# Bitcoin-Wildlife-Sanctuary/recursive-stwo

Hardware: AMD Instinct MI355X
Metric: recursive proofs verified/sec (higher is better)
Workload: dtype u32 (M31 modular integers)

## Files before the change

### recursive-stwo_amd/csrc/poseidon2.hpp

```cpp
#pragma once
#include "field.hpp"

namespace rsv {

struct State16 {
    uint32_t s[16];
};

#define RSV_RC_FULL_INIT { \
    {0x768bab52, 0x70e0ab7d, 0x3d266c8a, 0x6da42045, 0x600fef22, 0x41dace6b, 0x64f9bdd4, 0x5d42d4fe, \
     0x76b1516d, 0x6fc9a717, 0x70ac4fb6, 0x00194ef6, 0x22b644e2, 0x1f7916d5, 0x47581be2, 0x2710a123}, \
    {0x6284e867, 0x018d3afe, 0x5df99ef3, 0x4c1e467b, 0x566f6abc, 0x2994e427, 0x538a6d42, 0x5d7bf2cf, \
     0x7fda2dab, 0x0fd854c4, 0x46922fca, 0x3d7763a1, 0x19fd05ca, 0x0a4bbb43, 0x15075851, 0x3d903d76}, \
    {0x2d290ff7, 0x40809fa0, 0x59dac6ec, 0x127927a2, 0x6bbf0ea0, 0x0294140f, 0x24742976, 0x6e84c081, \
     0x22484f4a, 0x354cae59, 0x0453ffe1, 0x3f47a3cc, 0x0088204e, 0x6066e109, 0x3b7c4b80, 0x6b55665d}, \
    {0x3bc4b897, 0x735bf378, 0x508daf42, 0x1884fc2b, 0x7214f24c, 0x7498be0a, 0x1a60e640, 0x3303f928, \
     0x29b46376, 0x5c96bb68, 0x65d097a5, 0x1d358e9f, 0x4a9a9017, 0x4724cf76, 0x347af70f, 0x1e77e59a}, \
    {0x57090613, 0x1fa42108, 0x17bbef50, 0x1ff7e11c, 0x047b24ca, 0x4e140275, 0x4fa086f5, 0x079b309c, \
     0x1159bd47, 0x6d37e4e5, 0x075d8dce, 0x12121ca0, 0x7f6a7c40, 0x68e182ba, 0x5493201b, 0x0444a80e}, \
    {0x0064f4c6, 0x6467abe6, 0x66975762, 0x2af68f9b, 0x345b33be, 0x1b70d47f, 0x053db717, 0x381189cb, \
     0x43b915f8, 0x20df3694, 0x0f459d26, 0x77a0e97b, 0x2f73e739, 0x1876c2f9, 0x65a0e29a, 0x4cabefbe}, \
    {0x5abd1268, 0x4d34a760, 0x12771799, 0x69a0c9ac, 0x39091e55, 0x7f611cd0, 0x3af055da, 0x7ac0bbdf, \
     0x6e0f3a24, 0x41e3b6f7, 0x49b3756d, 0x568bc538, 0x20c079d8, 0x1701c72c, 0x7670dc6c, 0x5a439035}, \
    {0x7c93e00e, 0x561fbb4d, 0x1178907b, 0x02737406, 0x32fb24f1, 0x6323b60a, 0x6ab12418, 0x42c99cea, \
     0x155a0b97, 0x53d1c6aa, 0x2bd20347, 0x279b3d73, 0x4f5f3c70, 0x0245af6c, 0x238359d3, 0x49966a59}}
__constant__ __attribute__((aligned(64))) uint32_t RC_FULL[8][16] = RSV_RC_FULL_INIT;
constexpr uint32_t RC_FULL_K[8][16] = RSV_RC_FULL_INIT;

#define RSV_RC_PARTIAL_INIT { \
   0x7f7ec4bf, 0x0421926f, 0x5198e669, 0x34db3148, 0x4368bafd, \
                                        0x66685c7f, 0x78d3249a, 0x60187881, 0x76dad67a, 0x0690b437, \
                                        0x1ea95311, 0x40e5369a, 0x38f103fc, 0x1d226a21, 0, 0}
__constant__ __attribute__((aligned(64))) uint32_t RC_PARTIAL[16] = RSV_RC_PARTIAL_INIT;
constexpr uint32_t RC_PARTIAL_K[16] = RSV_RC_PARTIAL_INIT;

__device__ __forceinline__ uint32_t pow5_ref(uint32_t x) {
    uint32_t x2 = m_sqr(x);
    return m_mul(m_sqr(x2), x);
}

__device__ __forceinline__ void mds4_ref(uint32_t& x0, uint32_t& x1, uint32_t& x2, uint32_t& x3) {
    uint32_t t0 = m_add(x0, x1), t1 = m_add(x2, x3);
    uint32_t t2 = m_add(m_dbl(x1), t1), t3 = m_add(m_dbl(x3), t0);
    uint32_t t4 = m_add(m_shl(t1, 2), t3), t5 = m_add(m_shl(t0, 2), t2);
    x0 = m_add(t3, t5);
    x1 = t5;
    x2 = m_add(t2, t4);
    x3 = t4;
}

__device__ __forceinline__ void mds16_ref(uint32_t* s) {
#pragma unroll
    for (int g = 0; g < 4; g++) mds4_ref(s[4 * g], s[4 * g + 1], s[4 * g + 2], s[4 * g + 3]);
#pragma unroll
    for (int j = 0; j < 4; j++) {
        uint32_t sum = m_add(m_add(s[j], s[j + 4]), m_add(s[j + 8], s[j + 12]));
#pragma unroll
        for (int g = 0; g < 4; g++) s[4 * g + j] = m_add(s[4 * g + j], sum);
    }
}

template <bool PACE>
struct PermT {
    static __device__ __forceinline__ uint64_t add64(uint64_t a, uint64_t b) {
        uint64_t d;
        asm("v_lshl_add_u64 %0, %1, 0, %2" : "=v"(d) : "v"(a), "v"(b));
        return d;
    }
    template <int SH>
    static __device__ __forceinline__ uint64_t shl_add64(uint64_t a, uint64_t b) {
        uint64_t d;
        asm("v_lshl_add_u64 %0, %1, %3, %2" : "=v"(d) : "v"(a), "v"(b), "n"(SH));
        return d;
    }
    static __device__ __forceinline__ uint32_t opaque(uint32_t k) {
        uint32_t r;
        asm volatile("s_mov_b32 %0, %1" : "=s"(r) : "n"(k));
        return r;
    }
    static __device__ __forceinline__ uint64_t opaque64(uint64_t k) {
        return (uint64_t)opaque((uint32_t)(k >> 32)) << 32 | opaque((uint32_t)k);
    }
    static __device__ __forceinline__ uint64_t mul64(uint32_t a, uint32_t b_uniform) {
        uint64_t d, carry;
        if constexpr (PACE) asm("v_mad_u64_u32 %0, %1, %2, %3, 0\n\ts_nop 0" : "=v"(d), "=s"(carry) : "v"(a), "s"(b_uniform));
        else asm("v_mad_u64_u32 %0, %1, %2, %3, 0" : "=v"(d), "=s"(carry) : "v"(a), "s"(b_uniform));
        return d;
    }
    static __device__ __forceinline__ uint64_t mad64(uint32_t a, uint32_t b_uniform, uint64_t c) {
        uint64_t d, carry;
        if constexpr (PACE) asm("v_mad_u64_u32 %0, %1, %2, %3, %4\n\ts_nop 0" : "=v"(d), "=s"(carry) : "v"(a), "s"(b_uniform), "v"(c));
        else asm("v_mad_u64_u32 %0, %1, %2, %3, %4" : "=v"(d), "=s"(carry) : "v"(a), "s"(b_uniform), "v"(c));
        return d;
    }
    static __device__ __forceinline__ uint64_t mad64s(int32_t a, int32_t b, uint64_t c_uniform) {
        uint64_t d, carry;
        if constexpr (PACE) asm("v_mad_i64_i32 %0, %1, %2, %3, %4\n\ts_nop 0" : "=v"(d), "=s"(carry) : "v"(a), "v"(b), "s"(c_uniform));
        else asm("v_mad_i64_i32 %0, %1, %2, %3, %4" : "=v"(d), "=s"(carry) : "v"(a), "v"(b), "s"(c_uniform));
        return d;
    }
    static __device__ __forceinline__ uint64_t sqr64s(int32_t a, uint64_t c_uniform) {
        uint64_t d, carry;
        if constexpr (PACE) asm("v_mad_i64_i32 %0, %1, %2, %2, %3\n\ts_nop 0" : "=v"(d), "=s"(carry) : "v"(a), "s"(c_uniform));
        else asm("v_mad_i64_i32 %0, %1, %2, %2, %3" : "=v"(d), "=s"(carry) : "v"(a), "s"(c_uniform));
        return d;
    }
    static __device__ __forceinline__ uint32_t dbl32(uint32_t x) {
        uint32_t d;
        asm("v_add_u32 %0, %1, %1" : "=v"(d) : "v"(x));
        return d;
    }
    static __device__ __forceinline__ uint32_t fold2(uint64_t V) {
        uint32_t r = (uint32_t)(V >> 32) + ((uint32_t)V >> 1);
        return r;
    }

    static constexpr uint64_t KP = 0 - ((uint64_t)P << 32);
    static constexpr uint64_t KN = 0 - ((uint64_t)P << 31), KQ = (uint64_t)P << 31;
    struct SboxK {
        uint64_t kp, kn, kq;
    };
    static __device__ __forceinline__ SboxK sbox_k() { return {opaque64(KP), opaque64(KN), opaque64(KQ)}; }
    static constexpr uint32_t CENTRE = 1u << 30;
    static constexpr uint32_t centred(uint32_t rc) { return (uint32_t)(((uint64_t)rc + CENTRE) % P); }

    static __device__ __forceinline__ uint32_t pow5c(int32_t x, const SboxK& k) {
        const int32_t xx = (int32_t)dbl32((uint32_t)x);
        const int32_t s1 = (int32_t)fold2(mad64s(xx, x, k.kp));
        const uint64_t V2 = sqr64s(s1, k.kn);
        uint32_t c4 = __builtin_amdgcn_alignbit((uint32_t)(V2 >> 32), (uint32_t)V2, 31) + ((uint32_t)V2 & P);
        if constexpr (PACE) asm volatile("s_nop 0" : "+v"(c4));
        return fold2(mad64s(xx, (int32_t)c4, k.kq));
    }

    static __device__ __forceinline__ void mds4_2x(uint32_t k2, uint32_t k4, uint32_t x0, uint32_t x1, uint32_t x2, uint32_t x3,
                                            uint64_t& y0, uint64_t& y1, uint64_t& y2, uint64_t& y3) {
        uint64_t T0 = mad64(x0, k2, mul64(x1, k2));
        uint64_t T1 = mad64(x2, k2, mul64(x3, k2));
        uint64_t T2 = mad64(x1, k4, T1);
        uint64_t T3 = mad64(x3, k4, T0);
        uint64_t T4 = shl_add64<2>(T1, T3);
        uint64_t T5 = shl_add64<2>(T0, T2);
        y0 = add64(T3, T5);
        y1 = T5;
        y2 = add64(T2, T4);
        y3 = T4;
    }

    static __device__ __forceinline__ void mds16_2x(uint32_t k2, uint32_t k4, const uint32_t* s, uint64_t* V) {
    #pragma unroll
        for (int g = 0; g < 4; g++)
            mds4_2x(k2, k4, s[4 * g], s[4 * g + 1], s[4 * g + 2], s[4 * g + 3], V[4 * g], V[4 * g + 1], V[4 * g + 2], V[4 * g + 3]);
    #pragma unroll
        for (int j = 0; j < 4; j++) {
            uint64_t sum = add64(add64(V[j], V[j + 4]), add64(V[j + 8], V[j + 12]));
    #pragma unroll
            for (int g = 0; g < 4; g++) V[4 * g + j] = add64(V[4 * g + j], sum);
        }
    }

    static constexpr uint32_t HI_FULL = 160, HI_PARTIAL = 1u << 18;
    template <uint32_t RC, uint32_t HI>
    static __device__ __forceinline__ int32_t centre_rc(uint32_t t) {
        static_assert(HI < P - RC, "round constant too close to P for the fused reduction");
        constexpr uint32_t c = P - RC;
        static_assert((uint64_t)P + HI - c <= 0x7FFFFFFFull, "t - c leaves the int32 range");
        const int32_t a = (int32_t)(t - c);
        const uint32_t q = (uint32_t)(a >> 31) ^ 0xC0000000u;
        return (int32_t)((uint32_t)a + q);
    }

    template <int R, int I>
    static __device__ __forceinline__ void sbox_full(const uint64_t* V, uint32_t* s, const SboxK& k) {
        s[I] = pow5c(centre_rc<centred(RC_FULL_K[R][I]), HI_FULL>(fold2(V[I])), k);
        if constexpr (I + 1 < 16) sbox_full<R, I + 1>(V, s, k);
    }
    template <int I>
    static __device__ __forceinline__ void sbox_full4(uint32_t* s, const SboxK& k) {
        s[I] = pow5c(centre_rc<centred(RC_FULL_K[4][I]), HI_PARTIAL>(s[I]), k);
        if constexpr (I + 1 < 16) sbox_full4<I + 1>(s, k);
    }

    template <int R>
    static __device__ __forceinline__ void partial_round(uint32_t* s, uint32_t k2, uint32_t k6, const uint32_t* kd, const SboxK& k) {
        uint32_t u0 = pow5c(centre_rc<centred(RC_PARTIAL_K[R]), HI_PARTIAL>(s[0]), k);
        uint64_t a = mul64(u0, k2), b = mul64(s[1], k2);
    #pragma unroll
        for (int i = 2; i < 16; i += 2) { a = mad64(s[i], k2, a); b = mad64(s[i + 1], k2, b); }
        uint64_t sum2 = add64(a, b);
        s[0] = fold2(mad64(u0, k6, sum2));
    #pragma unroll
        for (int i = 1; i < 16; i++) s[i] = fold2(mad64(s[i], kd[i], sum2));
    }

    template <int R>
    static __device__ __forceinline__ void partial_pair(uint32_t* s, uint32_t k2, uint32_t k6, uint32_t k30, const uint32_t* kd,
                                                        const uint32_t* kq, const SboxK& k) {
        uint32_t u0 = pow5c(centre_rc<centred(RC_PARTIAL_K[R]), HI_PARTIAL>(s[0]), k);
        uint64_t a = mul64(u0, k2), b = mul64(s[1], k2);
    #pragma unroll
        for (int i = 2; i < 16; i += 2) { a = mad64(s[i], k2, a); b = mad64(s[i + 1], k2, b); }
        uint64_t sum2 = add64(a, b);
        const uint32_t s0 = fold2(mad64(u0, k6, sum2));
        const uint32_t sf = fold2(sum2);
        u0 = pow5c(centre_rc<centred(RC_PARTIAL_K[R + 1]), HI_PARTIAL>(s0), k);
        a = mul64(u0, k2); b = mul64(s[1], kd[1]);
    #pragma unroll
        for (int i = 2; i < 16; i += 2) { a = mad64(s[i], kd[i], a); b = mad64(s[i + 1], kd[i + 1], b); }
        a = mad64(sf, k30, a);
        sum2 = add64(a, b);
        s[0] = fold2(mad64(u0, k6, sum2));
    #pragma unroll
        for (int i = 1; i < 16; i++) s[i] = fold2(mad64(s[i], kq[i], mad64(sf, kd[i], sum2)));
    }

    static __device__ __forceinline__ void poseidon2_rounds(uint32_t* s, uint32_t k2, uint32_t k4) {
        uint64_t V[16];
        const uint32_t k6 = opaque(6);
        const SboxK k5 = sbox_k();
        mds16_2x(k2, k4, s, V);
        sbox_full<0, 0>(V, s, k5); mds16_2x(k2, k4, s, V);
        sbox_full<1, 0>(V, s, k5); mds16_2x(k2, k4, s, V);
        sbox_full<2, 0>(V, s, k5); mds16_2x(k2, k4, s, V);
        sbox_full<3, 0>(V, s, k5); mds16_2x(k2, k4, s, V);
    #pragma unroll
        for (int i = 0; i < 16; i++) s[i] = fold2(V[i]);
        uint32_t kd[16];
        kd[0] = k6;
    #define RSV_KD(i) kd[i] = opaque(4u << (i));
        RSV_KD(1) RSV_KD(2) RSV_KD(3) RSV_KD(4) RSV_KD(5) RSV_KD(6) RSV_KD(7) RSV_KD(8)
        RSV_KD(9) RSV_KD(10) RSV_KD(11) RSV_KD(12) RSV_KD(13) RSV_KD(14) RSV_KD(15)
    #undef RSV_KD
        uint32_t kq[16];
        kq[0] = 0;
    #pragma unroll
        for (int i = 1; i < 8; i++) kq[i] = kd[2 * i + 1];
    #define RSV_KQ(i) kq[i] = opaque(8u << (2 * (i)));
        RSV_KQ(8) RSV_KQ(9) RSV_KQ(10) RSV_KQ(11) RSV_KQ(12) RSV_KQ(13) RSV_KQ(14)
    #undef RSV_KQ
        kq[15] = k4;
        const uint32_t k30 = opaque(30);
        partial_round<0>(s, k2, k6, kd, k5);
        partial_pair<1>(s, k2, k6, k30, kd, kq, k5);  partial_pair<3>(s, k2, k6, k30, kd, kq, k5);  partial_pair<5>(s, k2, k6, k30, kd, kq, k5);
        partial_pair<7>(s, k2, k6, k30, kd, kq, k5);  partial_pair<9>(s, k2, k6, k30, kd, kq, k5);  partial_pair<11>(s, k2, k6, k30, kd, kq, k5);
        partial_round<13>(s, k2, k6, kd, k5);
        sbox_full4<0>(s, k5);      mds16_2x(k2, k4, s, V);
        sbox_full<5, 0>(V, s, k5); mds16_2x(k2, k4, s, V);
        sbox_full<6, 0>(V, s, k5); mds16_2x(k2, k4, s, V);
        sbox_full<7, 0>(V, s, k5);
    }

    static __device__ __forceinline__ void poseidon2_inline(uint32_t* s) {
        const uint32_t k2 = opaque(2), k4 = opaque(4);
        poseidon2_rounds(s, k2, k4);
        uint64_t V[16];
        mds16_2x(k2, k4, s, V);
    #pragma unroll
        for (int i = 0; i < 16; i++) {
            uint32_t t = fold2(V[i]);
            s[i] = min(t, t - P);
        }
    }

    template <bool HI>
    static __device__ __forceinline__ void poseidon2_inline_half(uint32_t* s, uint32_t* out8) {
        const uint32_t k2 = opaque(2), k4 = opaque(4);
        poseidon2_rounds(s, k2, k4);
        uint64_t V[16];
    #pragma unroll
        for (int g = 0; g < 4; g++)
            mds4_2x(k2, k4, s[4 * g], s[4 * g + 1], s[4 * g + 2], s[4 * g + 3], V[4 * g], V[4 * g + 1], V[4 * g + 2], V[4 * g + 3]);
        if constexpr (HI) {
    #pragma unroll
            for (int j = 0; j < 4; j++) {
                const uint64_t sum = add64(add64(V[j], V[j + 4]), add64(V[j + 8], V[j + 12]));
                const uint32_t t0 = fold2(add64(V[8 + j], sum)), t1 = fold2(add64(V[12 + j], sum));
                out8[j] = min(t0, t0 - P);
                out8[4 + j] = min(t1, t1 - P);
            }
        } else {
    #pragma unroll
            for (int j = 0; j < 4; j++) {
                const uint64_t sum = add64(add64(V[j], V[j + 4]), add64(V[j + 8], V[j + 12]));
                const uint32_t t0 = fold2(add64(V[j], sum)), t1 = fold2(add64(V[4 + j], sum));
                out8[j] = min(t0, t0 - P);
                out8[4 + j] = min(t1, t1 - P);
            }
        }
    }
};
__device__ __forceinline__ void poseidon2_inline(uint32_t* s) { PermT<true>::poseidon2_inline(s); }

#ifdef RSV_COUNT_PERMS
__device__ unsigned long long g_perm_counter[16];
__shared__ unsigned s_perm_tag;
#define RSV_TAG(k) do { if (threadIdx.x == 0) s_perm_tag = (k); __syncthreads(); } while (0)
__device__ __forceinline__ void count_perm_call() {
    const unsigned long long m = __ballot(1);
    if ((threadIdx.x & 63u) == (unsigned)__builtin_ctzll(m)) {
        atomicAdd(&g_perm_counter[2 * (s_perm_tag & 7u)], (unsigned long long)__builtin_popcountll(m));
        atomicAdd(&g_perm_counter[2 * (s_perm_tag & 7u) + 1], 1ull);
    }
}
#else
#define RSV_TAG(k) do { } while (0)
__device__ __forceinline__ void count_perm_call() {}
#endif

__device__ __noinline__ State16 poseidon2(State16 st) {
    count_perm_call();
    poseidon2_inline(st.s);
    return st;
}

struct Hash8 {
    uint32_t w[8];
};
__device__ __forceinline__ State16 join(const Hash8& l, const Hash8& r) {
    State16 st;
#pragma unroll
    for (int i = 0; i < 8; i++) { st.s[i] = l.w[i]; st.s[8 + i] = r.w[i]; }
    return st;
}
__device__ __forceinline__ Hash8 rate_of(const State16& st) {
    Hash8 h;
#pragma unroll
    for (int i = 0; i < 8; i++) h.w[i] = st.s[i];
    return h;
}
__device__ __forceinline__ Hash8 cap_of(const State16& st) {
    Hash8 h;
#pragma unroll
    for (int i = 0; i < 8; i++) h.w[i] = st.s[8 + i];
    return h;
}
__device__ __forceinline__ Hash8 zero8() {
    Hash8 h;
#pragma unroll
    for (int i = 0; i < 8; i++) h.w[i] = 0;
    return h;
}
template <bool HI, bool PACE>
__device__ __noinline__ Hash8 poseidon2_half_t(State16 st) {
    count_perm_call();
    Hash8 h;
    PermT<PACE>::template poseidon2_inline_half<HI>(st.s, h.w);
    return h;
}
struct RowRC {
    uint32_t f[8];
};
__device__ __forceinline__ RowRC load_row_rc(uint32_t i) {
    RowRC k;
#pragma unroll
    for (int r = 0; r < 8; r++) k.f[r] = RC_FULL[r][i];
    return k;
}
template <bool HI>
__device__ __noinline__ Hash8 poseidon2_row_half(State16 st);
__device__ __noinline__ State16 poseidon2_row_state(State16 st);
__shared__ uint32_t s_row_rc[8][16];
template <int PACE>
__device__ __forceinline__ void row_rc_init() {
    if constexpr (PACE == 2) {
        if (threadIdx.x < 128) s_row_rc[threadIdx.x >> 4][threadIdx.x & 15u] = RC_FULL[threadIdx.x >> 4][threadIdx.x & 15u];
        __syncthreads();
    }
}
constexpr int FORM_ROW = 2;
template <int PACE = 1>
__device__ __forceinline__ Hash8 poseidon2_half(State16 st, uint32_t hi) {
    if constexpr (PACE == FORM_ROW) return hi ? poseidon2_row_half<true>(st) : poseidon2_row_half<false>(st);
    else return hi ? poseidon2_half_t<true, PACE != 0>(st) : poseidon2_half_t<false, PACE != 0>(st);
}
template <int PACE = 1>
__device__ __forceinline__ State16 poseidon2_full(State16 st) {
    if constexpr (PACE == FORM_ROW) return poseidon2_row_state(st);
    else return poseidon2(st);
}
template <int PACE>
__device__ __forceinline__ uint32_t vlane() { return PACE == FORM_ROW ? threadIdx.x >> 4 : threadIdx.x; }
template <int PACE = 1>
__device__ __forceinline__ Hash8 perm_rate(const Hash8& l, const Hash8& r) { return poseidon2_half<PACE>(join(l, r), 0u); }
template <int PACE = 1>
__device__ __forceinline__ Hash8 perm_cap(const Hash8& l, const Hash8& r) { return poseidon2_half<PACE>(join(l, r), 1u); }
__device__ __forceinline__ bool hash_eq(const Hash8& a, const Hash8& b) {
    uint32_t d = 0;
#pragma unroll
    for (int i = 0; i < 8; i++) d |= a.w[i] ^ b.w[i];
    return d == 0;
}

}
```

Baseline: 2.207 million.

## Restructure Poseidon2 external MDS as column-sum plus per-group M4

Rewrites the 16-wide external MDS so the doubled column sums across the four groups are computed first. Each group then applies a multiply-free M4 (adds and shifts) to x*2 plus the column sum. The s-box of each group now runs right after that group's MDS, so only four 64-bit accumulators are live at a time instead of sixteen. The goal is fewer multiplies and lower register pressure in the full rounds. The cost is a different instruction mix and reliance on M4 being linear to keep the result identical.

Result: faster. 2.238 million (median of 6 runs) (+1.4%).

```diff
diff --git a/recursive-stwo_amd/csrc/poseidon2.hpp b/recursive-stwo_amd/csrc/poseidon2.hpp
--- a/recursive-stwo_amd/csrc/poseidon2.hpp
+++ b/recursive-stwo_amd/csrc/poseidon2.hpp
@@ -133,32 +133,28 @@
         return fold2(mad64s(xx, (int32_t)c4, k.kq));
     }
 
-    static __device__ __forceinline__ void mds4_2x(uint32_t k2, uint32_t k4, uint32_t x0, uint32_t x1, uint32_t x2, uint32_t x3,
-                                            uint64_t& y0, uint64_t& y1, uint64_t& y2, uint64_t& y3) {
-        uint64_t T0 = mad64(x0, k2, mul64(x1, k2));
-        uint64_t T1 = mad64(x2, k2, mul64(x3, k2));
-        uint64_t T2 = mad64(x1, k4, T1);
-        uint64_t T3 = mad64(x3, k4, T0);
-        uint64_t T4 = shl_add64<2>(T1, T3);
-        uint64_t T5 = shl_add64<2>(T0, T2);
-        y0 = add64(T3, T5);
-        y1 = T5;
-        y2 = add64(T2, T4);
-        y3 = T4;
-    }
-
-    static __device__ __forceinline__ void mds16_2x(uint32_t k2, uint32_t k4, const uint32_t* s, uint64_t* V) {
-    #pragma unroll
-        for (int g = 0; g < 4; g++)
-            mds4_2x(k2, k4, s[4 * g], s[4 * g + 1], s[4 * g + 2], s[4 * g + 3], V[4 * g], V[4 * g + 1], V[4 * g + 2], V[4 * g + 3]);
-    #pragma unroll
-        for (int j = 0; j < 4; j++) {
-            uint64_t sum = add64(add64(V[j], V[j + 4]), add64(V[j + 8], V[j + 12]));
-    #pragma unroll
-            for (int g = 0; g < 4; g++) V[4 * g + j] = add64(V[4 * g + j], sum);
+    static __device__ __forceinline__ void colsums_2x(uint32_t k2, const uint32_t* s, uint64_t* X2) {
+    #pragma unroll
+        for (int j = 0; j < 4; j++) X2[j] = mul64(s[j], k2);
+    #pragma unroll
+        for (int g = 1; g < 4; g++) {
+    #pragma unroll
+            for (int j = 0; j < 4; j++) X2[j] = mad64(s[4 * g + j], k2, X2[j]);
         }
     }
-
+    static __device__ __forceinline__ void mds4(uint64_t z0, uint64_t z1, uint64_t z2, uint64_t z3,
+                                                uint64_t& y0, uint64_t& y1, uint64_t& y2, uint64_t& y3) {
+        uint64_t t0 = add64(z0, z1), t1 = add64(z2, z3);
+        uint64_t t2 = shl_add64<1>(z1, t1), t3 = shl_add64<1>(z3, t0);
+        uint64_t t4 = shl_add64<2>(t1, t3), t5 = shl_add64<2>(t0, t2);
+        y0 = add64(t3, t5);
+        y1 = t5;
+        y2 = add64(t2, t4);
+        y3 = t4;
+    }
+    static __device__ __forceinline__ void mds_group_2x(uint32_t k2, const uint64_t* X2, const uint32_t* x, uint64_t* V) {
+        mds4(mad64(x[0], k2, X2[0]), mad64(x[1], k2, X2[1]), mad64(x[2], k2, X2[2]), mad64(x[3], k2, X2[3]), V[0], V[1], V[2], V[3]);
+    }
     static constexpr uint32_t HI_FULL = 160, HI_PARTIAL = 1u << 18;
     template <uint32_t RC, uint32_t HI>
     static __device__ __forceinline__ int32_t centre_rc(uint32_t t) {
@@ -170,10 +166,30 @@
         return (int32_t)((uint32_t)a + q);
     }
 
-    template <int R, int I>
+    template <int R, int I, int END = 16>
     static __device__ __forceinline__ void sbox_full(const uint64_t* V, uint32_t* s, const SboxK& k) {
         s[I] = pow5c(centre_rc<centred(RC_FULL_K[R][I]), HI_FULL>(fold2(V[I])), k);
-        if constexpr (I + 1 < 16) sbox_full<R, I + 1>(V, s, k);
+        if constexpr (I + 1 < END) sbox_full<R, I + 1, END>(V, s, k);
+    }
+    template <int R>
+    static __device__ __forceinline__ void mds_sbox(uint32_t k2, uint32_t* s, const SboxK& k) {
+        uint64_t X2[4], V[16];
+        colsums_2x(k2, s, X2);
+        mds_group_2x(k2, X2, s, V);           sbox_full<R, 0, 4>(V, s, k);
+        mds_group_2x(k2, X2, s + 4, V + 4);   sbox_full<R, 4, 8>(V, s, k);
+        mds_group_2x(k2, X2, s + 8, V + 8);   sbox_full<R, 8, 12>(V, s, k);
+        mds_group_2x(k2, X2, s + 12, V + 12); sbox_full<R, 12, 16>(V, s, k);
+    }
+    static __device__ __forceinline__ void mds_fold(uint32_t k2, uint32_t* s) {
+        uint64_t X2[4];
+        colsums_2x(k2, s, X2);
+    #pragma unroll
+        for (int g = 0; g < 4; g++) {
+            uint64_t V[4];
+            mds_group_2x(k2, X2, s + 4 * g, V);
+    #pragma unroll
+            for (int j = 0; j < 4; j++) s[4 * g + j] = fold2(V[j]);
+        }
     }
     template <int I>
     static __device__ __forceinline__ void sbox_full4(uint32_t* s, const SboxK& k) {
@@ -215,16 +231,13 @@
     }
 
     static __device__ __forceinline__ void poseidon2_rounds(uint32_t* s, uint32_t k2, uint32_t k4) {
-        uint64_t V[16];
         const uint32_t k6 = opaque(6);
         const SboxK k5 = sbox_k();
-        mds16_2x(k2, k4, s, V);
-        sbox_full<0, 0>(V, s, k5); mds16_2x(k2, k4, s, V);
-        sbox_full<1, 0>(V, s, k5); mds16_2x(k2, k4, s, V);
-        sbox_full<2, 0>(V, s, k5); mds16_2x(k2, k4, s, V);
-        sbox_full<3, 0>(V, s, k5); mds16_2x(k2, k4, s, V);
-    #pragma unroll
-        for (int i = 0; i < 16; i++) s[i] = fold2(V[i]);
+        mds_sbox<0>(k2, s, k5);
+        mds_sbox<1>(k2, s, k5);
+        mds_sbox<2>(k2, s, k5);
+        mds_sbox<3>(k2, s, k5);
+        mds_fold(k2, s);
         uint32_t kd[16];
         kd[0] = k6;
     #define RSV_KD(i) kd[i] = opaque(4u << (i));
@@ -244,47 +257,34 @@
         partial_pair<1>(s, k2, k6, k30, kd, kq, k5);  partial_pair<3>(s, k2, k6, k30, kd, kq, k5);  partial_pair<5>(s, k2, k6, k30, kd, kq, k5);
         partial_pair<7>(s, k2, k6, k30, kd, kq, k5);  partial_pair<9>(s, k2, k6, k30, kd, kq, k5);  partial_pair<11>(s, k2, k6, k30, kd, kq, k5);
         partial_round<13>(s, k2, k6, kd, k5);
-        sbox_full4<0>(s, k5);      mds16_2x(k2, k4, s, V);
-        sbox_full<5, 0>(V, s, k5); mds16_2x(k2, k4, s, V);
-        sbox_full<6, 0>(V, s, k5); mds16_2x(k2, k4, s, V);
-        sbox_full<7, 0>(V, s, k5);
+        sbox_full4<0>(s, k5);
+        mds_sbox<5>(k2, s, k5);
+        mds_sbox<6>(k2, s, k5);
+        mds_sbox<7>(k2, s, k5);
     }
 
     static __device__ __forceinline__ void poseidon2_inline(uint32_t* s) {
         const uint32_t k2 = opaque(2), k4 = opaque(4);
         poseidon2_rounds(s, k2, k4);
-        uint64_t V[16];
-        mds16_2x(k2, k4, s, V);
-    #pragma unroll
-        for (int i = 0; i < 16; i++) {
-            uint32_t t = fold2(V[i]);
-            s[i] = min(t, t - P);
-        }
+        mds_fold(k2, s);
+    #pragma unroll
+        for (int i = 0; i < 16; i++) s[i] = min(s[i], s[i] - P);
     }
 
     template <bool HI>
     static __device__ __forceinline__ void poseidon2_inline_half(uint32_t* s, uint32_t* out8) {
         const uint32_t k2 = opaque(2), k4 = opaque(4);
         poseidon2_rounds(s, k2, k4);
-        uint64_t V[16];
-    #pragma unroll
-        for (int g = 0; g < 4; g++)
-            mds4_2x(k2, k4, s[4 * g], s[4 * g + 1], s[4 * g + 2], s[4 * g + 3], V[4 * g], V[4 * g + 1], V[4 * g + 2], V[4 * g + 3]);
-        if constexpr (HI) {
+        uint64_t X2[4];
+        colsums_2x(k2, s, X2);
+    #pragma unroll
+        for (int g = 0; g < 2; g++) {
+            uint64_t V[4];
+            mds_group_2x(k2, X2, s + (HI ? 8 : 0) + 4 * g, V);
     #pragma unroll
             for (int j = 0; j < 4; j++) {
-                const uint64_t sum = add64(add64(V[j], V[j + 4]), add64(V[j + 8], V[j + 12]));
-                const uint32_t t0 = fold2(add64(V[8 + j], sum)), t1 = fold2(add64(V[12 + j], sum));
-                out8[j] = min(t0, t0 - P);
-                out8[4 + j] = min(t1, t1 - P);
-            }
-        } else {
-    #pragma unroll
-            for (int j = 0; j < 4; j++) {
-                const uint64_t sum = add64(add64(V[j], V[j + 4]), add64(V[j + 8], V[j + 12]));
-                const uint32_t t0 = fold2(add64(V[j], sum)), t1 = fold2(add64(V[4 + j], sum));
-                out8[j] = min(t0, t0 - P);
-                out8[4 + j] = min(t1, t1 - P);
+                const uint32_t t = fold2(V[j]);
+                out8[4 * g + j] = min(t, t - P);
             }
         }
     }
```
